# dphoyes/OpenCL-Structure-from-Motion

Hardware: AMD Instinct MI355X
Metric: stereo frame-pairs/sec (1242x375) through pushBack+matchFeatures(2), p_matched bit-exact (higher is better)
Workload: dtype u8

## Files before the change

### include/visomatch.h

```cpp
#ifndef VISOMATCH_H
#define VISOMATCH_H

#include <stdint.h>

#ifdef __cplusplus
extern "C" {
#endif

#define VSM_OK 0
#define VSM_EDIMS (-1)
#define VSM_ENOTREADY (-2)
#define VSM_EHIP (-3)
#define VSM_EARG (-4)

typedef struct vsm_handle vsm_handle;

typedef struct vsm_params {
  int32_t nms_n;
  int32_t nms_tau;
  int32_t match_binsize;
  int32_t match_radius;
  int32_t match_disp_tolerance;
  int32_t outlier_disp_tolerance;
  int32_t outlier_flow_tolerance;
// ... 155 lines not shown
int32_t vsm_host_ties(const int32_t *x, const int32_t *y, int32_t n, int32_t *pairs, int32_t cap);
int32_t vsm_debug_ties_gpu(const int32_t *x, const int32_t *y, int32_t n, int32_t *pairs, int32_t cap, double *kernel_us);

int32_t vsm_host_outliers_and_prior(const vsm_params *p, const vsm_p_match *list, int32_t n, int32_t method, vsm_p_match *out,
                                    int32_t cap, float *ranges, int32_t w, int32_t h);
int32_t vsm_host_outliers_and_prior_threads(const vsm_params *p, const vsm_p_match *list, int32_t n, int32_t method, vsm_p_match *out,
                                            int32_t cap, float *ranges, int32_t w, int32_t h, int32_t threads);
int32_t vsm_debug_dc2(const vsm_params *p, const vsm_p_match *list, int32_t n, int32_t method, int32_t gpu_ties, int32_t copies,
                      vsm_p_match *out, int32_t cap, float *ranges, int32_t w, int32_t h, double *kernel_us);
void vsm_debug_dc2_band_factor(int32_t f);
int32_t vsm_debug_predicates(const uint32_t *quads, int32_t n, int32_t *out);
int32_t vsm_debug_seq_plan(int32_t n_frames, int32_t pool_threads, int32_t host_in, int32_t seq_chunk, int32_t seq_first_chunk,
                           const char *plan, int32_t *chunk, int32_t *starts, int32_t cap);
int32_t vsm_debug_chunk_jobs(int32_t method, int32_t multi_stage, int32_t sides, int32_t banks, int32_t chunk, const int32_t *starts,
                             int32_t n_chunks, const int32_t *counts, const uint8_t *tr_valid, int32_t *frames_out, int32_t *max_nq_out);
int32_t vsm_debug_pair_jobs(int32_t method, int32_t multi_stage, int32_t sides, int32_t n_frames, const int32_t *counts, const int32_t *pairs,
                            int32_t n_pairs, int32_t chunk, const uint8_t *tr_valid, int32_t *pairs_out, int32_t *max_nq_out);
int32_t vsm_debug_refine(vsm_handle *h, int32_t method, const vsm_p_match *const *lists, const int32_t *counts, int32_t P,
                         vsm_p_match *const *out, int32_t *out_counts);
int32_t vsm_debug_refine_check(int32_t w, int32_t h, const vsm_p_match *const *lists, const int32_t *counts, int32_t P);
int32_t vsm_debug_parabolic_apply(const vsm_p_match *const *lists, const int32_t *const *records, const int32_t *counts, int32_t P,
                                  vsm_p_match *const *out, int32_t *out_counts);
int32_t vsm_host_parabolic_fits(const int32_t *records, int32_t n, float *uv, int32_t *ok);
int32_t vsm_debug_compact_keys(int32_t method, int32_t pass, int32_t P, const int32_t *n_query, const int32_t *const *flag,
                               const vsm_p_match *const *raw, const int32_t *key_cap, int32_t old_keys, vsm_p_match *const *list_out,
                               int32_t *count_out, uint64_t *const *keys_out);

typedef struct {
  vsm_params match;
  int32_t bucket_max_features;
  double bucket_width, bucket_height;
  double f, cu, cv;
  double base;
  int32_t ransac_iters;
  double inlier_threshold;
  int32_t reweighting;
} vsm_vo_stereo_params;
typedef struct vsm_vo_stereo vsm_vo_stereo;

void vsm_vo_stereo_default_params(vsm_vo_stereo_params *p);
vsm_vo_stereo *vsm_vo_stereo_create(const vsm_vo_stereo_params *p);
void vsm_vo_stereo_destroy(vsm_vo_stereo *v);
int vsm_vo_stereo_process(vsm_vo_stereo *v, const uint8_t *I1, const uint8_t *I2, int32_t width, int32_t height,
                          int32_t bpl, int replace);
int vsm_vo_stereo_process_device(vsm_vo_stereo *v, const uint8_t *dI1, const uint8_t *dI2, int32_t width,
                                 int32_t height, int32_t bpl, int replace);
// ... 88 lines not shown
```

### opencl-structure-from-motion_amd/csrc/vsm_api.cpp

```cpp
#include <math.h>
#include <stdio.h>
#include <stdlib.h>
#include <string.h>

#include <algorithm>
#include <chrono>
#include <memory>
#include <thread>
#include <unordered_map>
#include <vector>

#include "vsm_host.h"
#include "vsm_dc_gpu.h"
#include "vsm_internal.h"
#include "vsm_jobs.h"
#include "vsm_stage.h"
#include "vsm_tracks.h"
#include "vsm_points.h"
#include "vsm_resect.h"
#include "vsm_motions.h"

#define HIPCHK(expr)                                                                              \
  do {                                                                                            \
    hipError_t e_ = (expr);                                                                       \
    if (e_ != hipSuccess) {                                                                       \
      fprintf(stderr, "visomatch: HIP error %s at %s:%d (%s)\n", hipGetErrorString(e_), __FILE__, \
              __LINE__, #expr);                                                                   \
      return VSM_EHIP;                                                                            \
    }                                                                                             \
  } while (0)

static inline int32_t bpl16(int32_t w) { return w + 15 - (w - 1) % 16; }
static int cpu_budget() {
  unsigned hc = std::thread::hardware_concurrency();
  int budget = hc ? (int)hc : 8;
  if (FILE *f = fopen("/sys/fs/cgroup/cpu.max", "r")) {
    char q[64];
    long period = 0;
    if (fscanf(f, "%63s %ld", q, &period) == 2 && strcmp(q, "max") != 0 && period > 0) {
      long quota = atol(q);
      if (quota > 0) budget = std::min(budget, (int)std::max(1L, quota / period));
    }
    fclose(f);
// ... 1282 lines not shown
```

### opencl-structure-from-motion_amd/csrc/vsm_debug.inc

```

template <typename T>
struct DebugDev {
  T *p = nullptr;
  DebugDev() = default;
  DebugDev(const DebugDev &) = delete;
  DebugDev &operator=(const DebugDev &) = delete;
  ~DebugDev() {
    if (p) (void)hipFree(p);
  }
  bool alloc(size_t n) { return hipMalloc((void **)&p, std::max<size_t>(n, 1) * sizeof(T)) == hipSuccess; }
  operator T *() const { return p; }
};

struct DebugPairs {
  struct Pair {
    size_t raw = 0, flag = 0, blockcnt = 0, list1 = 0, list2 = 0, pf = 0;
    bool one_list = false;
    size_t keys = 0;
    int32_t key_cap = 0;
    int32_t count[2] = {0, 0};
    size_t n_in = 0;
    const vsm_p_match *raw_in = nullptr, *list2_in = nullptr;
    const int32_t *flag_in = nullptr, *pf_in = nullptr;
  };
// ... 623 lines not shown
int32_t vsm_debug_parabolic_apply(const vsm_p_match *const *lists, const int32_t *const *records, const int32_t *counts, int32_t P,
                                  vsm_p_match *const *out, int32_t *out_counts) {
  if (P < 1 || P > VSM_DEBUG_REFINE_MAX_PAIRS || !lists || !records || !counts || !out || !out_counts) return VSM_EARG;
  for (int32_t k = 0; k < P; k++)
    if (counts[k] < 0 || counts[k] > VSM_PARA_MAX_LIST || (counts[k] > 0 && (!lists[k] || !records[k]))) return VSM_EARG;
  DebugPairs D;
  HIPCHK(debug_lists_create(D, nullptr, lists, records, counts, P, true, VsmJob()));
  vsm_launch_parabolic_apply(nullptr, g_no_prof, D.d_pairs, P);
  HIPCHK(hipGetLastError());
  HIPCHK(hipDeviceSynchronize());
  HIPCHK(debug_lists_fetch(D, counts, P, true, out, out_counts));
  return VSM_OK;
}

int32_t vsm_host_parabolic_fits(const int32_t *records, int32_t n, float *uv, int32_t *ok) {
  if (n < 0 || (n > 0 && (!records || !uv || !ok))) return VSM_EARG;
  for (int32_t i = 0; i < n; i++) {
    const int32_t *r = records + (size_t)i * 12;
    ok[i] = vsm_host_parabolic_update(r + 3, r[1], r[2], uv[2 * i], uv[2 * i + 1]) ? 1 : 0;
  }
  return n;
}

}
```

### opencl-structure-from-motion_amd/csrc/vsm_dev.h

```cpp
#pragma once

#include "vsm_internal.h"

#define WAVE 64

#define VSM_AS1 __attribute__((address_space(1)))
typedef uint32_t vsm_u4 __attribute__((ext_vector_type(4)));
typedef int32_t vsm_i4 __attribute__((ext_vector_type(4)));
__device__ __forceinline__ uint4 ldg_u4(const void *p) {
  const vsm_u4 v = *(const VSM_AS1 vsm_u4 *)p;
  return make_uint4(v.x, v.y, v.z, v.w);
}
__device__ __forceinline__ int4 ldg_i4(const void *p) {
  const vsm_i4 v = *(const VSM_AS1 vsm_i4 *)p;
  return make_int4(v.x, v.y, v.z, v.w);
}
__device__ __forceinline__ uint4 ldg_u4_at(const void *base, uint32_t byte_off) {
  const vsm_u4 v = *(const VSM_AS1 vsm_u4 *)((const VSM_AS1 char *)base + byte_off);
  return make_uint4(v.x, v.y, v.z, v.w);
}
typedef uint32_t vsm_u4_a4 __attribute__((ext_vector_type(4), aligned(4)));
__device__ __forceinline__ uint4 ldg_u4_at_dw(const void *base, uint32_t byte_off) {
  const vsm_u4_a4 v = *(const VSM_AS1 vsm_u4_a4 *)((const VSM_AS1 char *)base + byte_off);
  return make_uint4(v.x, v.y, v.z, v.w);
}
__device__ __forceinline__ uint32_t ldg_u32_at(const void *base, uint32_t byte_off) {
  return *(const VSM_AS1 uint32_t *)((const VSM_AS1 char *)base + byte_off);
}
__device__ __forceinline__ int32_t ldg_i32(const void *p) { return *(const VSM_AS1 int32_t *)p; }
__device__ __forceinline__ uint32_t ldg_u32(const void *p) { return *(const VSM_AS1 uint32_t *)p; }

__device__ __forceinline__ int xcd_remap(int b, int nblocks) {
  const int per = (nblocks + 7) >> 3;
  return (b & 7) * per + (b >> 3);
// ... 53 lines not shown
```

### opencl-structure-from-motion_amd/csrc/vsm_match.hip

```cpp

#include <stdlib.h>

#include <algorithm>

#include "vsm_internal.h"
#include "vsm_dev.h"

#define VSM_MATCH_BLOCK 256
#define VSM_MATCH_WAVES 5
#define VSM_MATCH_GBIG 2
#define VSM_STEREO_BY_BIN 1

#ifdef VSM_MATCH_TIMING
#if VSM_MATCH_TIMING != 1 && VSM_MATCH_TIMING != 3
#error "VSM_MATCH_TIMING: 1 (cycles per stage and phase) or 3 (wave life on the device-wide clock)"
#endif
__device__ unsigned int vsm_mt_n;
__device__ unsigned int vsm_mt[1 << 18][8];
extern "C" int vsm_debug_match_timing(unsigned int *out, unsigned int cap, int reset) {
  unsigned int n = 0;
  if (hipMemcpyFromSymbol(&n, HIP_SYMBOL(vsm_mt_n), 4) != hipSuccess) return -1;
  if (n > (1u << 18)) n = 1u << 18;
  if (n > cap) n = cap;
  if (n && hipMemcpyFromSymbol(out, HIP_SYMBOL(vsm_mt), (size_t)n * 32) != hipSuccess) return -1;
  if (reset) {
    const unsigned int z = 0;
    if (hipMemcpyToSymbol(HIP_SYMBOL(vsm_mt_n), &z, 4) != hipSuccess) return -1;
  }
  return (int)n;
}
#if VSM_MATCH_TIMING == 1
#define MT_PHASE(k) const long long mt_ph##k = clock64()
#define MT_PHASE_ADD(ph)           \
// ... 587 lines not shown
}

__device__ __forceinline__ uint4 small_desc_tiled(const uint8_t *__restrict__ t, int bpl, int u, int v) {
#define TDU(x, y) ((uint32_t)t[vsm_tiled_at(bpl, (x), (y))])
#define TDV(x, y) ((uint32_t)t[vsm_tiled_at(bpl, (x), (y)) + VSM_TILED_DV])
  uint4 r;
  r.x = TDU(u, v - 2) | (TDU(u - 2, v - 1) << 8) | (TDU(u, v - 1) << 16) | (TDU(u + 2, v - 1) << 24);
  r.y = TDU(u - 1, v) | (TDU(u, v) << 8) | (TDU(u, v) << 16) | (TDU(u + 1, v) << 24);
  r.z = TDU(u - 2, v + 1) | (TDU(u, v + 1) << 8) | (TDU(u + 2, v + 1) << 16) | (TDU(u, v + 2) << 24);
  r.w = TDV(u, v - 1) | (TDV(u - 1, v) << 8) | (TDV(u + 1, v) << 16) | (TDV(u, v + 1) << 24);
#undef TDU
#undef TDV
  return r;
}

__device__ __forceinline__ uint32_t sad16(const uint4 &a, const uint4 &b) {
  uint32_t s = __builtin_amdgcn_sad_u8(a.x, b.x, 0u);
  s = __builtin_amdgcn_sad_u8(a.y, b.y, s);
  s = __builtin_amdgcn_sad_u8(a.z, b.z, s);
  return __builtin_amdgcn_sad_u8(a.w, b.w, s);
}

template <bool TILED>
__device__ __forceinline__ uint4 refine_ref_desc(const VsmImage &ref, const VsmDims &dc, int ru, int rv) {
  uint4 rd;
  const int b0 = (ru - 2) & ~3, rsh = 8 * ((ru - 2) - b0);
  uint64_t wu[5], wv[3];
  if (TILED) {
    const int j0 = b0 >> 2;
#pragma unroll
    for (int r = 0; r < 5; r++) {
      const uint8_t *row = ref.duv_tiled;
      const uint32_t lo = ldg_u32(row + vsm_tiled_at(dc.bpl, 4 * j0, rv - 2 + r)), hi = ldg_u32(row + vsm_tiled_at(dc.bpl, 4 * j0 + 4, rv - 2 + r));
      wu[r] = ((((uint64_t)hi) << 32) | lo) >> rsh;
      if (r >= 1 && r <= 3) {
        const uint32_t lv = ldg_u32(row + vsm_tiled_at(dc.bpl, 4 * j0, rv - 2 + r) + VSM_TILED_DV), hv = ldg_u32(row + vsm_tiled_at(dc.bpl, 4 * j0 + 4, rv - 2 + r) + VSM_TILED_DV);
        wv[r - 1] = ((((uint64_t)hv) << 32) | lv) >> rsh;
      }
    }
  } else {
#pragma unroll
    for (int r = 0; r < 5; r++) {
      const uint32_t *pr = (const uint32_t *)(ref.du_full + (size_t)(rv - 2 + r) * dc.bpl + b0);
      wu[r] = ((((uint64_t)pr[1]) << 32) | pr[0]) >> rsh;
    }
#pragma unroll
    for (int r = 0; r < 3; r++) {
      const uint32_t *pr = (const uint32_t *)(ref.dv_full + (size_t)(rv - 1 + r) * dc.bpl + b0);
      wv[r] = ((((uint64_t)pr[1]) << 32) | pr[0]) >> rsh;
    }
  }
#define WB(w, c) ((uint32_t)((w) >> (8 * (c))) & 0xffu)
  rd.x = WB(wu[0], 2) | (WB(wu[1], 0) << 8) | (WB(wu[1], 2) << 16) | (WB(wu[1], 4) << 24);
  rd.y = WB(wu[2], 1) | (WB(wu[2], 2) << 8) | (WB(wu[2], 2) << 16) | (WB(wu[2], 3) << 24);
  rd.z = WB(wu[3], 0) | (WB(wu[3], 2) << 8) | (WB(wu[3], 4) << 16) | (WB(wu[4], 2) << 24);
  rd.w = WB(wv[0], 2) | (WB(wv[1], 1) << 8) | (WB(wv[1], 3) << 16) | (WB(wv[2], 2) << 24);
#undef WB
  return rd;
}

template <bool TILED>
__global__ void __launch_bounds__(256)
    k_refine(const VsmImage *__restrict__ imgs, const VsmPair *__restrict__ pairs, const VsmJob *__restrict__ jobs,
             VsmJob job0, VsmDims dp, VsmDims dc, int method, int nbx, int npairs) {
  const int lb = xcd_remap(blockIdx.x, gridDim.x);
  const int pj = lb / nbx, bx = lb - pj * nbx;
  if (pj >= npairs) return;
  const VsmJob &jb = jobs ? jobs[pj] : job0;
  const VsmPair &pair = pairs[pj];
  const int g = bx * blockDim.x + threadIdx.x;
  const int mi = g / 3, step = g - mi * 3;
  const VsmImage &ref = imgs[jb.img_curr];
  uint4 rd;
  {
    const int lane = threadIdx.x & 63;
    const int first_mi = (g - lane) / 3, rmi = first_mi + lane;
    uint4 mine = make_uint4(0, 0, 0, 0);
    if (lane < 22 && rmi < pair.count[1]) {
      const vsm_p_match *rm = pair.list2 + rmi;
      mine = refine_ref_desc<TILED>(ref, dc, (int)rm->u1c, (int)rm->v1c);
    }
    const int src = mi - first_mi;
    rd.x = (uint32_t)__shfl((int)mine.x, src, 64);
    rd.y = (uint32_t)__shfl((int)mine.y, src, 64);
    rd.z = (uint32_t)__shfl((int)mine.z, src, 64);
    rd.w = (uint32_t)__shfl((int)mine.w, src, 64);
  }
  if (mi >= pair.count[1]) return;
  if (step == 0 && !(method == 0 || method == 2)) return;
  if (step == 1 && !(method == 1 || method == 2)) return;
  if (step == 2 && method != 2) return;
  vsm_p_match *m = pair.list2 + mi;
  const VsmImage &tgt = step == 0 ? imgs[jb.img_prev] : (step == 1 ? imgs[jb.img_curr + 1] : imgs[jb.img_prev + 1]);
  const VsmDims &dt = step == 1 ? dc : dp;
  float *pu = step == 0 ? &m->u1p : (step == 1 ? &m->u2c : &m->u2p);
  float *pv = pu + 1;
  const float u2 = *pu, v2 = *pv;
  if (u2 - 2 < VSM_MARGIN || u2 + 2 > dt.w - 1 - VSM_MARGIN || v2 - 2 < VSM_MARGIN || v2 + 2 > dt.h - 1 - VSM_MARGIN)
    return;
  const int iu = (int)u2, iv = (int)v2;
  uint32_t U[9][3], V[9][3];
  if (TILED) {
    const int o = (iu - 4) & 7, b = o >> 2;
    const uint32_t sb = (uint32_t)(o & 3);
#pragma unroll
    for (int r = 0; r < 9; r++) {
      const uint8_t *pr = tgt.duv_tiled + vsm_tiled_at(dt.bpl, (iu - 4) & ~7, iv - 4 + r);
      const uint4 t0 = ldg_u4(pr), t1 = ldg_u4(pr + 128);
      const uint32_t d0 = b ? t0.z : t0.x, d1 = b ? t1.x : t0.z, d2 = b ? t1.z : t1.x;
      U[r][0] = __builtin_amdgcn_alignbyte(d1, d0, sb);
      U[r][1] = __builtin_amdgcn_alignbyte(d2, d1, sb);
      U[r][2] = d2 >> (8 * sb);
      const uint32_t e0 = b ? t0.w : t0.y, e1 = b ? t1.y : t0.w, e2 = b ? t1.w : t1.y;
      V[r][0] = __builtin_amdgcn_alignbyte(e1, e0, sb);
      V[r][1] = __builtin_amdgcn_alignbyte(e2, e1, sb);
      V[r][2] = e2 >> (8 * sb);
    }
  } else {
    const int a0 = (iu - 4) & ~3, sh = 8 * ((iu - 4) - a0);
#pragma unroll
    for (int r = 0; r < 9; r++) {
      const uint32_t *pr = (const uint32_t *)(tgt.du_full + (size_t)(iv - 4 + r) * dt.bpl + a0);
      const uint32_t d0 = pr[0], d1 = pr[1], d2 = pr[2];
      U[r][0] = (uint32_t)((((uint64_t)d1 << 32) | d0) >> sh);
      U[r][1] = (uint32_t)((((uint64_t)d2 << 32) | d1) >> sh);
      U[r][2] = d2 >> sh;
      if (r >= 1 && r <= 7) {
        const uint32_t *qr = (const uint32_t *)(tgt.dv_full + (size_t)(iv - 4 + r) * dt.bpl + a0);
        const uint32_t e0 = qr[0], e1 = qr[1], e2 = qr[2];
        V[r][0] = (uint32_t)((((uint64_t)e1 << 32) | e0) >> sh);
        V[r][1] = (uint32_t)((((uint64_t)e2 << 32) | e1) >> sh);
        V[r][2] = e2 >> sh;
      } else {
        V[r][0] = V[r][1] = V[r][2] = 0;
      }
    }
  }
#define UB(r, c) ((U[(r)][(c) >> 2] >> (8 * ((c)&3))) & 0xffu)
#define VB(r, c) ((V[(r)][(c) >> 2] >> (8 * ((c)&3))) & 0xffu)
  uint32_t best = 0xffffffffu;
  int ind = 0;
#pragma unroll
  for (int ddv = 0; ddv < 5; ddv++) {
#pragma unroll
    for (int ddu = 0; ddu < 5; ddu++) {
      const int r = ddv + 2, c = ddu + 2;
      uint4 t;
      t.x = UB(r - 2, c) | (UB(r - 1, c - 2) << 8) | (UB(r - 1, c) << 16) | (UB(r - 1, c + 2) << 24);
      t.y = UB(r, c - 1) | (UB(r, c) << 8) | (UB(r, c) << 16) | (UB(r, c + 1) << 24);
      t.z = UB(r + 1, c - 2) | (UB(r + 1, c) << 8) | (UB(r + 1, c + 2) << 16) | (UB(r + 2, c) << 24);
      t.w = VB(r - 1, c) | (VB(r, c - 1) << 8) | (VB(r, c + 1) << 16) | (VB(r + 1, c) << 24);
      const uint32_t cost = sad16(rd, t);
      if (cost < best) {
        best = cost;
        ind = ddv * 5 + ddu;
      }
    }
  }
#undef UB
#undef VB
  *pu = (float)((double)u2 + ((double)(float)(ind % 5) - 2.0));
  *pv = (float)((double)v2 + ((double)(float)(ind / 5) - 2.0));
}

__global__ void __launch_bounds__(256)
    k_parabolic_costs(const VsmImage *__restrict__ imgs, const VsmPair *__restrict__ pairs,
                      const VsmJob *__restrict__ jobs, VsmJob job0, VsmDims dp, VsmDims dc, int method) {
  const VsmJob &jb = jobs ? jobs[blockIdx.y] : job0;
  const VsmPair &pair = pairs[blockIdx.y];
  const int img_prev = jb.img_prev, img_curr = jb.img_curr;
  const int lane = threadIdx.x & 63;
  const int g = (blockIdx.x * blockDim.x + threadIdx.x) >> 6;
  const int mi = g / 3, step = g - mi * 3;
  if (mi >= pair.count[1]) return;
  int32_t *out = pair.pf + ((size_t)mi * 3 + step) * 12;
  bool active = !((step == 0 && !(method == 0 || method == 2)) || (step == 1 && !(method == 1 || method == 2)) ||
                  (step == 2 && method != 2));
  if (!active) {
    if (lane == 0) out[0] = 2;
    return;
  }
  const vsm_p_match *m = pair.list2 + mi;
  const VsmImage &ref = imgs[img_curr];
  const VsmImage &tgt = step == 0 ? imgs[img_prev] : (step == 1 ? imgs[img_curr + 1] : imgs[img_prev + 1]);
  const VsmDims &dt = step == 1 ? dc : dp;
// ... 259 lines not shown

void vsm_launch_export_xy(hipStream_t s, const VsmPair *d_pairs, uint32_t *dst_host_mapped, int n_upper) {
  hipLaunchKernelGGL(k_export_xy, dim3(max(min(cdiv(n_upper, 256), 64), 1)), dim3(256), 0, s, d_pairs, dst_host_mapped);
}

void vsm_launch_parabolic_apply(hipStream_t s, VsmProf &pf, const VsmPair *d_pairs, int npairs) {
  if (npairs <= 0) return;
  static const VsmParaPlan plan = make_para_plan();
  pf.begin(VSM_K_PARA_APPLY, s);
  hipLaunchKernelGGL(k_parabolic_apply, dim3(npairs), dim3(1024), 0, s, d_pairs, plan);
  pf.end(s);
}

void vsm_launch_refine(hipStream_t s, VsmProf &pf, const VsmImage *d_imgs, const VsmPair *d_pairs, const VsmJob *d_jobs,
                       const VsmJob &job0, int npairs, const VsmDims &dp, const VsmDims &dc, int method, int refinement,
                       int n_upper) {
  if (n_upper <= 0) return;
  pf.begin(VSM_K_REFINE, s);
  if (refinement == 2)
    hipLaunchKernelGGL(k_parabolic_costs, dim3(cdiv(n_upper * 3 * 64, 256), npairs), dim3(256), 0, s, d_imgs, d_pairs,
                       d_jobs, job0, dp, dc, method);
  else
  {
    const int nbx = cdiv(n_upper * 3, 256), tot = ((nbx * npairs + 7) / 8) * 8;
    if (dc.scale == 2)
      hipLaunchKernelGGL(k_refine<true>, dim3(tot), dim3(256), 0, s, d_imgs, d_pairs, d_jobs, job0, dp, dc, method, nbx, npairs);
    else
      hipLaunchKernelGGL(k_refine<false>, dim3(tot), dim3(256), 0, s, d_imgs, d_pairs, d_jobs, job0, dp, dc, method, nbx, npairs);
  }
  pf.end(s);
}
```

### opencl-structure-from-motion_amd/visomatch.py

```python
import ctypes as C
import os

import numpy as np

HERE = os.path.dirname(os.path.abspath(__file__))
os.environ.setdefault("GPU_MAX_HW_QUEUES", "5")
LIB_PATH = os.environ.get("VSM_LIB_PATH") or os.path.join(HERE, "libvisomatch.so")

P_MATCH = np.dtype(
    [("u1p", "<f4"), ("v1p", "<f4"), ("i1p", "<i4"), ("u2p", "<f4"), ("v2p", "<f4"), ("i2p", "<i4"),
     ("u1c", "<f4"), ("v1c", "<f4"), ("i1c", "<i4"), ("u2c", "<f4"), ("v2c", "<f4"), ("i2c", "<i4")])
assert P_MATCH.itemsize == 48

INT_PARAMS = ["nms_n", "nms_tau", "match_binsize", "match_radius", "match_disp_tolerance",
              "outlier_disp_tolerance", "outlier_flow_tolerance", "multi_stage", "half_resolution", "refinement"]
TRACKS_WAVE_MAX = 64
TRACKS_BLOCK_MAX = 2048
FEATURE_SETS = {"1p1": 0, "2p1": 1, "1c1": 2, "2c1": 3, "1p2": 4, "2p2": 5, "1c2": 6, "2c2": 7}

EXPORTS = ["vsm_default_params", "vsm_create", "vsm_destroy", "vsm_set_intrinsics", "vsm_push_back",
           "vsm_push_back_device", "vsm_wait_for_stream", "vsm_match", "vsm_num_matches", "vsm_get_matches", "vsm_bucket", "vsm_gain",
           "vsm_num_features", "vsm_get_features", "vsm_set_stage_capture", "vsm_stage_size", "vsm_stage_get",
           "vsm_num_ranges", "vsm_get_ranges", "vsm_get_gradients", "vsm_get_filter_responses", "vsm_get_counters",
           "vsm_get_timings", "vsm_set_profiling", "vsm_num_kernels", "vsm_kernel_name", "vsm_get_kernel_stats",
           "vsm_host_delaunay", "vsm_host_delaunay_split", "vsm_debug_delaunay_gpu", "vsm_debug_dc_bench", "vsm_host_ties", "vsm_debug_ties_gpu", "vsm_host_outliers_and_prior", "vsm_host_outliers_and_prior_threads", "vsm_debug_dc2", "vsm_debug_dc2_band_factor", "vsm_debug_predicates", "vsm_debug_seq_plan", "vsm_debug_chunk_jobs", "vsm_debug_pair_jobs", "vsm_debug_refine", "vsm_debug_refine_check", "vsm_debug_parabolic_apply", "vsm_host_parabolic_fits", "vsm_debug_compact_keys", "vsm_local_cpus", "vsm_forkjoin_cpus", "vsm_device_pool_stats", "vsm_device_pool_trim", "vsm_sequence_run", "vsm_sequence_num_matches", "vsm_sequence_get_matches",
           "vsm_sequence_get_timings", "vsm_sequence_path", "vsm_pairs_run", "vsm_pairs_num_matches", "vsm_pairs_get_matches", "vsm_pairs_get_timings",
           "vsm_tracks_run", "vsm_pairs_tracks", "vsm_tracks_count", "vsm_tracks_num_obs", "vsm_tracks_get", "vsm_tracks_of_matches",
           "vsm_tracks_get_stats", "vsm_tracks_get_timings", "vsm_host_tracks",
           "vsm_triangulate_default_params", "vsm_triangulate_run", "vsm_tracks_triangulate", "vsm_points_count", "vsm_points_get",
           "vsm_points_get_stats", "vsm_points_get_timings", "vsm_host_triangulate",
           "vsm_resect_default_params", "vsm_resect_run", "vsm_points_resect", "vsm_resect_count", "vsm_resect_get", "vsm_resect_get_stats",
           "vsm_resect_get_timings", "vsm_host_resect", "vsm_set_option", "vsm_version", "vsm_host_register", "vsm_host_unregister",
           "vsm_multi_create", "vsm_multi_destroy", "vsm_multi_process", "vsm_multi_num_sequences", "vsm_multi_get_motion",
           "vsm_multi_motion_valid", "vsm_multi_num_matches", "vsm_multi_get_matches", "vsm_multi_num_inliers", "vsm_multi_get_inliers",
           "vsm_multi_get_timings",
           "vsm_vo_stereo_default_params", "vsm_vo_stereo_create", "vsm_vo_stereo_destroy", "vsm_vo_stereo_process",
           "vsm_vo_stereo_process_device", "vsm_vo_stereo_process_matches", "vsm_vo_stereo_get_motion",
           "vsm_vo_stereo_motion_valid", "vsm_vo_stereo_num_matches", "vsm_vo_stereo_get_matches",
           "vsm_vo_stereo_num_inliers", "vsm_vo_stereo_get_inliers", "vsm_vo_stereo_gain", "vsm_vo_stereo_matcher",
           "vsm_vo_stereo_get_timings", "vsm_vo_sampler_seed", "vsm_host_estimate_motion_stereo",
           "vsm_vo_mono_default_params", "vsm_vo_mono_create", "vsm_vo_mono_destroy", "vsm_vo_mono_process",
           "vsm_vo_mono_process_device", "vsm_vo_mono_process_matches", "vsm_vo_mono_get_motion",
           "vsm_vo_mono_motion_valid", "vsm_vo_mono_num_matches", "vsm_vo_mono_get_matches", "vsm_vo_mono_num_inliers",
           "vsm_vo_mono_get_inliers", "vsm_vo_mono_gain", "vsm_vo_mono_matcher", "vsm_vo_mono_get_timings",
           "vsm_vo_mono_device_svd", "vsm_vo_mono_device_stages",
           "vsm_debug_mono_fit", "vsm_debug_mono_count", "vsm_debug_mono_triangulate", "vsm_debug_mono_vote",
           "vsm_host_estimate_motion_mono",
           "vsm_motions_run", "vsm_pairs_motions", "vsm_motions_count", "vsm_motions_get", "vsm_motions_inliers", "vsm_motions_matches",
# ... 106 lines not shown
        L.vsm_kernel_name.argtypes = [i32]
        L.vsm_get_kernel_stats.argtypes = [vp, vp, vp]
        L.vsm_host_delaunay.argtypes = [vp, vp, i32, vp, i32, i32]
        L.vsm_host_delaunay_split.argtypes = [vp, vp, i32, vp, i32, i32, i32]
        L.vsm_debug_delaunay_gpu.argtypes = [vp, vp, i32, vp, i32, i32, i32, i32]
        L.vsm_debug_dc_bench.argtypes = [vp, vp, i32, i32, i32, i32, i32, i32]
        L.vsm_debug_dc_bench.restype = C.c_double
        L.vsm_host_ties.argtypes = [vp, vp, i32, vp, i32]
        L.vsm_debug_ties_gpu.argtypes = [vp, vp, i32, vp, i32, vp]
        L.vsm_host_outliers_and_prior.argtypes = [C.POINTER(VsmParams), vp, i32, i32, vp, i32, vp, i32, i32]
        L.vsm_host_outliers_and_prior_threads.argtypes = [C.POINTER(VsmParams), vp, i32, i32, vp, i32, vp, i32, i32, i32]
        L.vsm_debug_dc2.argtypes = [C.POINTER(VsmParams), vp, i32, i32, i32, i32, vp, i32, vp, i32, i32, vp]
        L.vsm_debug_dc2_band_factor.argtypes = [i32]
        L.vsm_debug_predicates.argtypes = [vp, i32, vp]
        L.vsm_debug_seq_plan.argtypes = [i32, i32, i32, i32, i32, C.c_char_p, vp, vp, i32]
        L.vsm_debug_chunk_jobs.restype = i32
        L.vsm_debug_chunk_jobs.argtypes = [i32, i32, i32, i32, i32, vp, i32, vp, vp, vp, vp]
        L.vsm_debug_pair_jobs.restype = i32
        L.vsm_debug_pair_jobs.argtypes = [i32, i32, i32, i32, vp, vp, i32, i32, vp, vp, vp]
        L.vsm_debug_refine.argtypes = [vp, i32, vp, vp, i32, vp, vp]
        L.vsm_debug_refine_check.argtypes = [i32, i32, vp, vp, i32]
        L.vsm_debug_parabolic_apply.argtypes = [vp, vp, vp, i32, vp, vp]
        L.vsm_host_parabolic_fits.argtypes = [vp, i32, vp, vp]
        L.vsm_debug_compact_keys.argtypes = [i32, i32, i32, vp, vp, vp, vp, i32, vp, vp, vp]
        L.vsm_pairs_run.argtypes = [vp, vp, vp, C.c_int64, C.c_int, i32, i32, i32, i32, i32, vp, i32, vp, vp]
        L.vsm_pairs_num_matches.argtypes = [vp, i32]
        L.vsm_pairs_get_matches.argtypes = [vp, i32, vp, i32]
        L.vsm_pairs_get_timings.argtypes = [vp, vp]
        L.vsm_pairs_get_timings.restype = None
        L.vsm_tracks_run.argtypes = [vp, i32, vp, i32, vp, vp, i32, i32]
        L.vsm_pairs_tracks.argtypes = [vp, i32, i32]
        L.vsm_tracks_count.argtypes = [vp]
        L.vsm_tracks_num_obs.argtypes = [vp]
        L.vsm_tracks_get.argtypes = [vp, vp, vp, vp]
        L.vsm_tracks_of_matches.argtypes = [vp, i32, vp, i32]
        L.vsm_tracks_get_stats.argtypes = [vp, vp]
        L.vsm_tracks_get_stats.restype = None
        L.vsm_tracks_get_timings.argtypes = [vp, vp]
        L.vsm_tracks_get_timings.restype = None
        L.vsm_host_tracks.restype = i32
        L.vsm_host_tracks.argtypes = [i32, vp, i32, vp, vp, i32, i32, vp, vp, vp, vp, vp]
        f64 = C.c_double
        L.vsm_triangulate_default_params.argtypes = [C.POINTER(VsmTriangulateParams)]
        L.vsm_triangulate_default_params.restype = None
        L.vsm_triangulate_run.argtypes = [vp, i32, vp, vp, f64, f64, f64, i32, vp, vp, vp, vp, C.POINTER(VsmTriangulateParams)]
        L.vsm_tracks_triangulate.argtypes = [vp, vp, vp, vp, vp, f64, f64, f64, C.POINTER(VsmTriangulateParams)]
# ... 611 lines not shown


def device_parabolic_apply(lists, records, counts=None):
    ms, cnt, ptrs = _refine_inputs(lists)
    rs = [np.ascontiguousarray(r, dtype=np.int32).reshape(-1, 3, 12) for r in records]
    assert len(rs) == len(ms) and all(len(r) == len(m) for r, m in zip(rs, ms))
    rptrs = (C.c_void_p * max(len(rs), 1))(*[r.ctypes.data if len(r) else None for r in rs])
    if counts is not None:
        cnt = np.ascontiguousarray(counts, dtype=np.int32)
    outs, oc, optrs = _refine_outputs([len(m) for m in ms])
    _check(lib().vsm_debug_parabolic_apply(ptrs, rptrs, _ptr(cnt), len(ms), optrs, _ptr(oc)), "vsm_debug_parabolic_apply")
    return [o[:n].copy() for o, n in zip(outs, oc)]


def host_parabolic_fits(records, uv):
    r = np.ascontiguousarray(records, dtype=np.int32).reshape(-1, 12)
    out = np.array(uv, dtype=np.float32).reshape(-1, 2).copy()
    assert len(out) == len(r)
    ok = np.zeros(len(r), dtype=np.int32)
    _check(lib().vsm_host_parabolic_fits(_ptr(r), len(r), _ptr(out), _ptr(ok)), "vsm_host_parabolic_fits")
    return out, ok


COMPACT_KEY_GUARD = 8


def device_compact_keys(flags, raws, key_caps, method=2, pass_=1, old_keys=False):
    fs = [np.ascontiguousarray(f, dtype=np.int32) for f in flags]
    rs = [np.ascontiguousarray(r, dtype=P_MATCH) for r in raws]
    assert len(fs) == len(rs) == len(key_caps) and all(len(f) == len(r) for f, r in zip(fs, rs))
    nq = np.array([len(f) for f in fs], dtype=np.int32)
    caps = np.ascontiguousarray(key_caps, dtype=np.int32)
    lists = [np.zeros(len(f) + 1, dtype=P_MATCH) for f in fs]
    keys = [np.zeros(int(c) + COMPACT_KEY_GUARD, dtype=np.uint64) for c in caps]
    counts = np.full(len(fs), -1, dtype=np.int32)
    tab = lambda arrs: (C.c_void_p * len(arrs))(*[a.ctypes.data for a in arrs])
    _check(lib().vsm_debug_compact_keys(int(method), int(pass_), len(fs), _ptr(nq), tab(fs), tab(rs), _ptr(caps), int(old_keys), tab(lists),
                                        _ptr(counts), tab(keys)), "vsm_debug_compact_keys")
    return [(l, int(n), k) for l, n, k in zip(lists, counts, keys)]


def local_cpus():
    buf = (C.c_int32 * 1024)()
    n = lib().vsm_local_cpus(C.cast(buf, C.c_void_p), 1024)
    return [int(buf[i]) for i in range(min(n, 1024))]

# ... 640 lines not shown
```

Measured before the change: 55750.

## Restructure refine kernel into per-wave steps with shared reference descriptors

Rewrites k_refine so that each block handles 64 matches, with one wave per refinement step and an extra wave that builds the reference descriptor into shared memory. The old scheme used a thread per (match, step) and shuffled the reference descriptors across lanes. Descriptor assembly now uses byte-permute helpers in a shared header, and the costs are computed first with a packed key min-reduction. It also adds a host reference path for testing. The intent is to cut per-thread index math and divergence and to use fewer instructions for packing. The trade-offs are a __syncthreads, one whole wave per block spent only on the reference, and a waves_per_eu constraint.

```diff
diff --git a/include/visomatch.h b/include/visomatch.h
--- a/include/visomatch.h
+++ b/include/visomatch.h
@@ -201,6 +201,9 @@
 int32_t vsm_debug_parabolic_apply(const vsm_p_match *const *lists, const int32_t *const *records, const int32_t *counts, int32_t P,
                                   vsm_p_match *const *out, int32_t *out_counts);
 int32_t vsm_host_parabolic_fits(const int32_t *records, int32_t n, float *uv, int32_t *ok);
+int32_t vsm_host_refine_forms(const uint8_t *du, const uint8_t *dv, const uint8_t *ref_du, const uint8_t *ref_dv, const int32_t *phase,
+                              const int32_t *ref_phase, int32_t n, int32_t *costs, int32_t *index);
+int32_t vsm_debug_refine_group(void);
 int32_t vsm_debug_compact_keys(int32_t method, int32_t pass, int32_t P, const int32_t *n_query, const int32_t *const *flag,
                                const vsm_p_match *const *raw, const int32_t *key_cap, int32_t old_keys, vsm_p_match *const *list_out,
                                int32_t *count_out, uint64_t *const *keys_out);
diff --git a/opencl-structure-from-motion_amd/csrc/vsm_api.cpp b/opencl-structure-from-motion_amd/csrc/vsm_api.cpp
--- a/opencl-structure-from-motion_amd/csrc/vsm_api.cpp
+++ b/opencl-structure-from-motion_amd/csrc/vsm_api.cpp
@@ -19,6 +19,7 @@
 #include "vsm_points.h"
 #include "vsm_resect.h"
 #include "vsm_motions.h"
+#include "vsm_refine.h"
 
 #define HIPCHK(expr)                                                                              \
   do {                                                                                            \
diff --git a/opencl-structure-from-motion_amd/csrc/vsm_debug.inc b/opencl-structure-from-motion_amd/csrc/vsm_debug.inc
--- a/opencl-structure-from-motion_amd/csrc/vsm_debug.inc
+++ b/opencl-structure-from-motion_amd/csrc/vsm_debug.inc
@@ -669,4 +669,32 @@
   return n;
 }
 
-}
+int32_t vsm_debug_refine_group(void) { return VR_GROUP; }
+
+int32_t vsm_host_refine_forms(const uint8_t *du, const uint8_t *dv, const uint8_t *ref_du, const uint8_t *ref_dv, const int32_t *phase,
+                              const int32_t *ref_phase, int32_t n, int32_t *costs, int32_t *index) {
+  if (n < 0 || (n > 0 && (!du || !dv || !ref_du || !ref_dv || !phase || !ref_phase || !costs || !index))) return VSM_EARG;
+  for (int32_t i = 0; i < n; i++)
+    if (phase[i] < 0 || phase[i] > 7 || ref_phase[i] < 0 || ref_phase[i] > 3) return VSM_EARG;
+  auto dword = [](const uint8_t *p) { return (uint32_t)p[0] | ((uint32_t)p[1] << 8) | ((uint32_t)p[2] << 16) | ((uint32_t)p[3] << 24); };
+  for (int32_t i = 0; i < n; i++) {
+    uint32_t U[9][3], V[9][3], RU[5][3], RV[5][3];
+    for (int r = 0; r < 9; r++) {
+      const uint8_t *pu = du + ((size_t)i * 9 + r) * 16, *pv = dv + ((size_t)i * 9 + r) * 16;
+      const uint32_t t0[4] = {dword(pu), dword(pv), dword(pu + 4), dword(pv + 4)}, t1[4] = {dword(pu + 8), dword(pv + 8), dword(pu + 12), dword(pv + 12)};
+      vr_tile_row(t0, t1, phase[i], U[r], V[r]);
+    }
+    for (int r = 0; r < 5; r++) {
+      const uint8_t *pu = ref_du + ((size_t)i * 5 + r) * 8, *pv = ref_dv + ((size_t)i * 5 + r) * 8;
+      vr_ref_row(dword(pu), dword(pu + 4), (uint32_t)ref_phase[i], RU[r]);
+      vr_ref_row(dword(pv), dword(pv + 4), (uint32_t)ref_phase[i], RV[r]);
+    }
+    uint32_t cost[25];
+    vr_costs(U, V, vr_ref_desc(RU, RV), cost);
+    for (int k = 0; k < 25; k++) costs[(size_t)i * 25 + k] = (int32_t)cost[k];
+    index[i] = vr_first_min(cost);
+  }
+  return n;
+}
+
+}
diff --git a/opencl-structure-from-motion_amd/csrc/vsm_dev.h b/opencl-structure-from-motion_amd/csrc/vsm_dev.h
--- a/opencl-structure-from-motion_amd/csrc/vsm_dev.h
+++ b/opencl-structure-from-motion_amd/csrc/vsm_dev.h
@@ -10,6 +10,11 @@
 __device__ __forceinline__ uint4 ldg_u4(const void *p) {
   const vsm_u4 v = *(const VSM_AS1 vsm_u4 *)p;
   return make_uint4(v.x, v.y, v.z, v.w);
+}
+typedef uint32_t vsm_u2 __attribute__((ext_vector_type(2)));
+__device__ __forceinline__ uint2 ldg_u2_at(const void *base, uint32_t byte_off) {
+  const vsm_u2 v = *(const VSM_AS1 vsm_u2 *)((const VSM_AS1 char *)base + byte_off);
+  return make_uint2(v.x, v.y);
 }
 __device__ __forceinline__ int4 ldg_i4(const void *p) {
   const vsm_i4 v = *(const VSM_AS1 vsm_i4 *)p;
diff --git a/opencl-structure-from-motion_amd/csrc/vsm_match.hip b/opencl-structure-from-motion_amd/csrc/vsm_match.hip
--- a/opencl-structure-from-motion_amd/csrc/vsm_match.hip
+++ b/opencl-structure-from-motion_amd/csrc/vsm_match.hip
@@ -5,10 +5,12 @@
 
 #include "vsm_internal.h"
 #include "vsm_dev.h"
+#include "vsm_refine.h"
 
 #define VSM_MATCH_BLOCK 256
 #define VSM_MATCH_WAVES 5
 #define VSM_MATCH_GBIG 2
+#define VSM_REFINE_WAVES 5
 #define VSM_STEREO_BY_BIN 1
 
 #ifdef VSM_MATCH_TIMING
@@ -642,145 +644,112 @@
 }
 
 template <bool TILED>
-__device__ __forceinline__ uint4 refine_ref_desc(const VsmImage &ref, const VsmDims &dc, int ru, int rv) {
-  uint4 rd;
-  const int b0 = (ru - 2) & ~3, rsh = 8 * ((ru - 2) - b0);
-  uint64_t wu[5], wv[3];
+__device__ __forceinline__ VrDesc refine_reference(const VsmImage &ref, const VsmDims &dc, int ru, int rv) {
+  const int b0 = (ru - 2) & ~3;
+  const uint32_t sb = (uint32_t)((ru - 2) - b0);
+  uint32_t U[5][3], V[5][3];
   if (TILED) {
-    const int j0 = b0 >> 2;
 #pragma unroll
     for (int r = 0; r < 5; r++) {
-      const uint8_t *row = ref.duv_tiled;
-      const uint32_t lo = ldg_u32(row + vsm_tiled_at(dc.bpl, 4 * j0, rv - 2 + r)), hi = ldg_u32(row + vsm_tiled_at(dc.bpl, 4 * j0 + 4, rv - 2 + r));
-      wu[r] = ((((uint64_t)hi) << 32) | lo) >> rsh;
-      if (r >= 1 && r <= 3) {
-        const uint32_t lv = ldg_u32(row + vsm_tiled_at(dc.bpl, 4 * j0, rv - 2 + r) + VSM_TILED_DV), hv = ldg_u32(row + vsm_tiled_at(dc.bpl, 4 * j0 + 4, rv - 2 + r) + VSM_TILED_DV);
-        wv[r - 1] = ((((uint64_t)hv) << 32) | lv) >> rsh;
-      }
+      const uint2 lo = ldg_u2_at(ref.duv_tiled, (uint32_t)vsm_tiled_at(dc.bpl, b0, rv - 2 + r)),
+                  hi = ldg_u2_at(ref.duv_tiled, (uint32_t)vsm_tiled_at(dc.bpl, b0 + 4, rv - 2 + r));
+      vr_ref_row(lo.x, hi.x, sb, U[r]);
+      vr_ref_row(lo.y, hi.y, sb, V[r]);
     }
   } else {
 #pragma unroll
     for (int r = 0; r < 5; r++) {
-      const uint32_t *pr = (const uint32_t *)(ref.du_full + (size_t)(rv - 2 + r) * dc.bpl + b0);
-      wu[r] = ((((uint64_t)pr[1]) << 32) | pr[0]) >> rsh;
-    }
-#pragma unroll
-    for (int r = 0; r < 3; r++) {
-      const uint32_t *pr = (const uint32_t *)(ref.dv_full + (size_t)(rv - 1 + r) * dc.bpl + b0);
-      wv[r] = ((((uint64_t)pr[1]) << 32) | pr[0]) >> rsh;
-    }
-  }
-#define WB(w, c) ((uint32_t)((w) >> (8 * (c))) & 0xffu)
-  rd.x = WB(wu[0], 2) | (WB(wu[1], 0) << 8) | (WB(wu[1], 2) << 16) | (WB(wu[1], 4) << 24);
-  rd.y = WB(wu[2], 1) | (WB(wu[2], 2) << 8) | (WB(wu[2], 2) << 16) | (WB(wu[2], 3) << 24);
-  rd.z = WB(wu[3], 0) | (WB(wu[3], 2) << 8) | (WB(wu[3], 4) << 16) | (WB(wu[4], 2) << 24);
-  rd.w = WB(wv[0], 2) | (WB(wv[1], 1) << 8) | (WB(wv[1], 3) << 16) | (WB(wv[2], 2) << 24);
-#undef WB
-  return rd;
+      const uint32_t at = (uint32_t)((rv - 2 + r) * dc.bpl + b0);
+      vr_ref_row(ldg_u32_at(ref.du_full, at), ldg_u32_at(ref.du_full, at + 4), sb, U[r]);
+      if (r >= 1 && r <= 3)
+        vr_ref_row(ldg_u32_at(ref.dv_full, at), ldg_u32_at(ref.dv_full, at + 4), sb, V[r]);
+      else
+        V[r][0] = V[r][1] = V[r][2] = 0;
+    }
+  }
+  return vr_ref_desc(U, V);
 }
 
 template <bool TILED>
-__global__ void __launch_bounds__(256)
+__device__ __forceinline__ void refine_window(const VsmImage &tgt, int bpl, int iu, int iv, uint32_t (&U)[9][3], uint32_t (&V)[9][3]) {
+  if (TILED) {
+    const int o = (iu - 4) & 7;
+    uint4 t0[9], t1[9];
+#pragma unroll
+    for (int r = 0; r < 9; r++) {
+      const uint32_t at = (uint32_t)vsm_tiled_at(bpl, (iu - 4) & ~7, iv - 4 + r);
+      t0[r] = ldg_u4_at(tgt.duv_tiled, at), t1[r] = ldg_u4_at(tgt.duv_tiled, at + 128);
+    }
+    __builtin_amdgcn_sched_barrier(0);
+#pragma unroll
+    for (int r = 0; r < 9; r++) {
+      const uint32_t a[4] = {t0[r].x, t0[r].y, t0[r].z, t0[r].w}, b[4] = {t1[r].x, t1[r].y, t1[r].z, t1[r].w};
+      vr_tile_row(a, b, o, U[r], V[r]);
+    }
+  } else {
+    const int a0 = (iu - 4) & ~3;
+    const uint32_t sb = (uint32_t)((iu - 4) - a0);
+#pragma unroll
+    for (int r = 0; r < 9; r++) {
+      const uint32_t at = (uint32_t)((iv - 4 + r) * bpl + a0);
+      vr_window_row(ldg_u32_at(tgt.du_full, at), ldg_u32_at(tgt.du_full, at + 4), ldg_u32_at(tgt.du_full, at + 8), sb, U[r]);
+      if (r >= 1 && r <= 7)
+        vr_window_row(ldg_u32_at(tgt.dv_full, at), ldg_u32_at(tgt.dv_full, at + 4), ldg_u32_at(tgt.dv_full, at + 8), sb, V[r]);
+      else
+        V[r][0] = V[r][1] = V[r][2] = 0;
+    }
+  }
+}
+
+template <bool TILED>
+__global__ void __launch_bounds__(256) __attribute__((amdgpu_waves_per_eu(VSM_REFINE_WAVES, VSM_REFINE_WAVES)))
     k_refine(const VsmImage *__restrict__ imgs, const VsmPair *__restrict__ pairs, const VsmJob *__restrict__ jobs,
              VsmJob job0, VsmDims dp, VsmDims dc, int method, int nbx, int npairs) {
+  __shared__ uint4 s_rd[VR_GROUP];
   const int lb = xcd_remap(blockIdx.x, gridDim.x);
   const int pj = lb / nbx, bx = lb - pj * nbx;
   if (pj >= npairs) return;
-  const VsmJob &jb = jobs ? jobs[pj] : job0;
+  const int img_prev = jobs ? jobs[pj].img_prev : job0.img_prev, img_curr = jobs ? jobs[pj].img_curr : job0.img_curr;
   const VsmPair &pair = pairs[pj];
-  const int g = bx * blockDim.x + threadIdx.x;
-  const int mi = g / 3, step = g - mi * 3;
-  const VsmImage &ref = imgs[jb.img_curr];
-  uint4 rd;
-  {
-    const int lane = threadIdx.x & 63;
-    const int first_mi = (g - lane) / 3, rmi = first_mi + lane;
-    uint4 mine = make_uint4(0, 0, 0, 0);
-    if (lane < 22 && rmi < pair.count[1]) {
-      const vsm_p_match *rm = pair.list2 + rmi;
-      mine = refine_ref_desc<TILED>(ref, dc, (int)rm->u1c, (int)rm->v1c);
-    }
-    const int src = mi - first_mi;
-    rd.x = (uint32_t)__shfl((int)mine.x, src, 64);
-    rd.y = (uint32_t)__shfl((int)mine.y, src, 64);
-    rd.z = (uint32_t)__shfl((int)mine.z, src, 64);
-    rd.w = (uint32_t)__shfl((int)mine.w, src, 64);
-  }
-  if (mi >= pair.count[1]) return;
-  if (step == 0 && !(method == 0 || method == 2)) return;
-  if (step == 1 && !(method == 1 || method == 2)) return;
-  if (step == 2 && method != 2) return;
-  vsm_p_match *m = pair.list2 + mi;
-  const VsmImage &tgt = step == 0 ? imgs[jb.img_prev] : (step == 1 ? imgs[jb.img_curr + 1] : imgs[jb.img_prev + 1]);
-  const VsmDims &dt = step == 1 ? dc : dp;
-  float *pu = step == 0 ? &m->u1p : (step == 1 ? &m->u2c : &m->u2p);
-  float *pv = pu + 1;
-  const float u2 = *pu, v2 = *pv;
-  if (u2 - 2 < VSM_MARGIN || u2 + 2 > dt.w - 1 - VSM_MARGIN || v2 - 2 < VSM_MARGIN || v2 + 2 > dt.h - 1 - VSM_MARGIN)
-    return;
-  const int iu = (int)u2, iv = (int)v2;
+  const int count = pair.count[1];
+  if (bx * VR_GROUP >= count) return;
+  const int lane = threadIdx.x & 63, wv = __builtin_amdgcn_readfirstlane(threadIdx.x >> 6);
+  const int nsteps = method == 2 ? 3 : 1;
+  const int step = method == 2 ? wv : method;
+  const int mi = bx * VR_GROUP + lane;
+  const bool live = mi < count;
+  vsm_p_match *m = pair.list2 + (live ? mi : count - 1);
+  float u2 = 0.f, v2 = 0.f;
+  bool ok = false;
   uint32_t U[9][3], V[9][3];
-  if (TILED) {
-    const int o = (iu - 4) & 7, b = o >> 2;
-    const uint32_t sb = (uint32_t)(o & 3);
-#pragma unroll
-    for (int r = 0; r < 9; r++) {
-      const uint8_t *pr = tgt.duv_tiled + vsm_tiled_at(dt.bpl, (iu - 4) & ~7, iv - 4 + r);
-      const uint4 t0 = ldg_u4(pr), t1 = ldg_u4(pr + 128);
-      const uint32_t d0 = b ? t0.z : t0.x, d1 = b ? t1.x : t0.z, d2 = b ? t1.z : t1.x;
-      U[r][0] = __builtin_amdgcn_alignbyte(d1, d0, sb);
-      U[r][1] = __builtin_amdgcn_alignbyte(d2, d1, sb);
-      U[r][2] = d2 >> (8 * sb);
-      const uint32_t e0 = b ? t0.w : t0.y, e1 = b ? t1.y : t0.w, e2 = b ? t1.w : t1.y;
-      V[r][0] = __builtin_amdgcn_alignbyte(e1, e0, sb);
-      V[r][1] = __builtin_amdgcn_alignbyte(e2, e1, sb);
-      V[r][2] = e2 >> (8 * sb);
-    }
+  if (wv == nsteps) {
+    const uint4 p1 = ldg_u4((const uint8_t *)m + 16);
+    const VrDesc d = refine_reference<TILED>(imgs[img_curr], dc, (int)__uint_as_float(p1.z), (int)__uint_as_float(p1.w));
+    s_rd[lane] = make_uint4(d.a0, d.b, d.a1, d.x);
   } else {
-    const int a0 = (iu - 4) & ~3, sh = 8 * ((iu - 4) - a0);
-#pragma unroll
-    for (int r = 0; r < 9; r++) {
-      const uint32_t *pr = (const uint32_t *)(tgt.du_full + (size_t)(iv - 4 + r) * dt.bpl + a0);
-      const uint32_t d0 = pr[0], d1 = pr[1], d2 = pr[2];
-      U[r][0] = (uint32_t)((((uint64_t)d1 << 32) | d0) >> sh);
-      U[r][1] = (uint32_t)((((uint64_t)d2 << 32) | d1) >> sh);
-      U[r][2] = d2 >> sh;
-      if (r >= 1 && r <= 7) {
-        const uint32_t *qr = (const uint32_t *)(tgt.dv_full + (size_t)(iv - 4 + r) * dt.bpl + a0);
-        const uint32_t e0 = qr[0], e1 = qr[1], e2 = qr[2];
-        V[r][0] = (uint32_t)((((uint64_t)e1 << 32) | e0) >> sh);
-        V[r][1] = (uint32_t)((((uint64_t)e2 << 32) | e1) >> sh);
-        V[r][2] = e2 >> sh;
-      } else {
-        V[r][0] = V[r][1] = V[r][2] = 0;
-      }
-    }
-  }
-#define UB(r, c) ((U[(r)][(c) >> 2] >> (8 * ((c)&3))) & 0xffu)
-#define VB(r, c) ((V[(r)][(c) >> 2] >> (8 * ((c)&3))) & 0xffu)
-  uint32_t best = 0xffffffffu;
-  int ind = 0;
-#pragma unroll
-  for (int ddv = 0; ddv < 5; ddv++) {
-#pragma unroll
-    for (int ddu = 0; ddu < 5; ddu++) {
-      const int r = ddv + 2, c = ddu + 2;
-      uint4 t;
-      t.x = UB(r - 2, c) | (UB(r - 1, c - 2) << 8) | (UB(r - 1, c) << 16) | (UB(r - 1, c + 2) << 24);
-      t.y = UB(r, c - 1) | (UB(r, c) << 8) | (UB(r, c) << 16) | (UB(r, c + 1) << 24);
-      t.z = UB(r + 1, c - 2) | (UB(r + 1, c) << 8) | (UB(r + 1, c + 2) << 16) | (UB(r + 2, c) << 24);
-      t.w = VB(r - 1, c) | (VB(r, c - 1) << 8) | (VB(r, c + 1) << 16) | (VB(r + 1, c) << 24);
-      const uint32_t cost = sad16(rd, t);
-      if (cost < best) {
-        best = cost;
-        ind = ddv * 5 + ddu;
-      }
-    }
-  }
-#undef UB
-#undef VB
-  *pu = (float)((double)u2 + ((double)(float)(ind % 5) - 2.0));
-  *pv = (float)((double)v2 + ((double)(float)(ind / 5) - 2.0));
+    if (step == 1) {
+      const uint4 p2 = ldg_u4((const uint8_t *)m + 32);
+      u2 = __uint_as_float(p2.y), v2 = __uint_as_float(p2.z);
+    } else {
+      const uint4 p0 = ldg_u4((const uint8_t *)m), p1 = ldg_u4((const uint8_t *)m + 16);
+      u2 = __uint_as_float(step == 0 ? p0.x : p0.w), v2 = __uint_as_float(step == 0 ? p0.y : p1.x);
+    }
+    const int tw = step == 1 ? dc.w : dp.w, th = step == 1 ? dc.h : dp.h, tbpl = step == 1 ? dc.bpl : dp.bpl;
+    ok = !(u2 - 2 < VSM_MARGIN || u2 + 2 > tw - 1 - VSM_MARGIN || v2 - 2 < VSM_MARGIN || v2 + 2 > th - 1 - VSM_MARGIN);
+    if (ok) refine_window<TILED>(imgs[step == 0 ? img_prev : (step == 1 ? img_curr + 1 : img_prev + 1)], tbpl, (int)u2, (int)v2, U, V);
+  }
+  __syncthreads();
+  if (wv == nsteps) return;
+  const uint4 q = s_rd[lane];
+  const VrDesc rd = {q.x, q.y, q.z, q.w};
+  uint32_t cost[25];
+  vr_costs(U, V, rd, cost);
+  const int ind = vr_first_min(cost);
+  if (live && ok) {
+    float *pu = step == 0 ? &m->u1p : (step == 1 ? &m->u2c : &m->u2p);
+    pu[0] = (float)((double)u2 + ((double)(float)(ind % 5) - 2.0));
+    pu[1] = (float)((double)v2 + ((double)(float)(ind / 5) - 2.0));
+  }
 }
 
 __global__ void __launch_bounds__(256)
@@ -1086,11 +1055,11 @@
                        d_jobs, job0, dp, dc, method);
   else
   {
-    const int nbx = cdiv(n_upper * 3, 256), tot = ((nbx * npairs + 7) / 8) * 8;
+    const int nbx = cdiv(n_upper, VR_GROUP), tot = ((nbx * npairs + 7) / 8) * 8, threads = 64 * ((method == 2 ? 3 : 1) + 1);
     if (dc.scale == 2)
-      hipLaunchKernelGGL(k_refine<true>, dim3(tot), dim3(256), 0, s, d_imgs, d_pairs, d_jobs, job0, dp, dc, method, nbx, npairs);
+      hipLaunchKernelGGL(k_refine<true>, dim3(tot), dim3(threads), 0, s, d_imgs, d_pairs, d_jobs, job0, dp, dc, method, nbx, npairs);
     else
-      hipLaunchKernelGGL(k_refine<false>, dim3(tot), dim3(256), 0, s, d_imgs, d_pairs, d_jobs, job0, dp, dc, method, nbx, npairs);
+      hipLaunchKernelGGL(k_refine<false>, dim3(tot), dim3(threads), 0, s, d_imgs, d_pairs, d_jobs, job0, dp, dc, method, nbx, npairs);
   }
   pf.end(s);
 }
diff --git a/opencl-structure-from-motion_amd/csrc/vsm_refine.h b/opencl-structure-from-motion_amd/csrc/vsm_refine.h
--- /dev/null
+++ b/opencl-structure-from-motion_amd/csrc/vsm_refine.h
@@ -0,0 +1,104 @@
+#pragma once
+
+#include "vsm_feat.h"
+
+#define VR_GROUP 64
+
+VF_HD uint32_t vr_sad(uint32_t a, uint32_t b, uint32_t acc) {
+#if defined(__HIP_DEVICE_COMPILE__)
+  return __builtin_amdgcn_sad_u8(a, b, acc);
+#else
+  for (int k = 0; k < 4; k++) {
+    const int x = (int)((a >> (8 * k)) & 0xffu), y = (int)((b >> (8 * k)) & 0xffu);
+    acc += (uint32_t)(x > y ? x - y : y - x);
+  }
+  return acc;
+#endif
+}
+
+struct VrDesc {
+  uint32_t a0, b, a1, x;
+};
+
+VF_HD void vr_window_row(uint32_t d0, uint32_t d1, uint32_t d2, uint32_t sb, uint32_t (&W)[3]) {
+  W[0] = vf_alignbyte(d1, d0, sb);
+  W[1] = vf_alignbyte(d2, d1, sb);
+  W[2] = d2 >> (8 * sb);
+}
+
+VF_HD void vr_tile_row(const uint32_t (&t0)[4], const uint32_t (&t1)[4], int o, uint32_t (&U)[3], uint32_t (&V)[3]) {
+  const bool b = (o >> 2) != 0;
+  const uint32_t sb = (uint32_t)(o & 3);
+  vr_window_row(b ? t0[2] : t0[0], b ? t1[0] : t0[2], b ? t1[2] : t1[0], sb, U);
+  vr_window_row(b ? t0[3] : t0[1], b ? t1[1] : t0[3], b ? t1[3] : t1[1], sb, V);
+}
+
+VF_HD void vr_ref_row(uint32_t lo, uint32_t hi, uint32_t sb, uint32_t (&W)[3]) {
+  W[0] = vf_alignbyte(hi, lo, sb);
+  W[1] = hi >> (8 * sb);
+  W[2] = 0;
+}
+
+VF_HD uint32_t vr_pick(const uint32_t (&W)[3], int c0, int c1, int c2, int c3) {
+#define VR_DW(c) ((c) < 0 ? 2 : (c) >> 2)
+#define VR_SEL(c, k) (((c) < 0 ? 0x0cu : (uint32_t)((c)-4 * lo)) << (8 * (k)))
+  const int l01 = VR_DW(c0) < VR_DW(c1) ? VR_DW(c0) : VR_DW(c1), l23 = VR_DW(c2) < VR_DW(c3) ? VR_DW(c2) : VR_DW(c3);
+  const int lo = l01 < l23 ? l01 : l23;
+  const uint32_t sel = VR_SEL(c0, 0) | VR_SEL(c1, 1) | VR_SEL(c2, 2) | VR_SEL(c3, 3);
+#undef VR_DW
+#undef VR_SEL
+  return lo == 0 ? vf_perm(W[1], W[0], sel) : (lo == 1 ? vf_perm(W[2], W[1], sel) : vf_perm(W[2], W[2], sel));
+}
+
+template <int ROWS>
+VF_HD uint32_t vr_form_a(const uint32_t (&U)[ROWS][3], const uint32_t (&V)[ROWS][3], int R, int c) {
+  return vf_perm(V[R][c >> 2], vr_pick(U[R], c - 2, c, c + 2, -1), 0x00020100u | ((uint32_t)(4 + (c & 3)) << 24));
+}
+template <int ROWS>
+VF_HD uint32_t vr_form_b(const uint32_t (&U)[ROWS][3], int R, int c) {
+  return vr_pick(U[R], c - 1, c, c, c + 1);
+}
+template <int ROWS>
+VF_HD uint32_t vr_form_x(const uint32_t (&U)[ROWS][3], const uint32_t (&V)[ROWS][3], int r, int c) {
+  const uint32_t col = (uint32_t)(c & 3);
+  return vf_perm(U[r + 2][c >> 2], U[r - 2][c >> 2], 0x0c0c0000u | ((4 + col) << 8) | col) | vr_pick(V[r], -1, -1, c - 1, c + 1);
+}
+
+template <int ROWS>
+VF_HD VrDesc vr_desc(const uint32_t (&U)[ROWS][3], const uint32_t (&V)[ROWS][3], int r, int c) {
+  VrDesc d;
+  d.a0 = vr_form_a<ROWS>(U, V, r - 1, c);
+  d.b = vr_form_b<ROWS>(U, r, c);
+  d.a1 = vr_form_a<ROWS>(U, V, r + 1, c);
+  d.x = vr_form_x<ROWS>(U, V, r, c);
+  return d;
+}
+
+VF_HD VrDesc vr_ref_desc(const uint32_t (&U)[5][3], const uint32_t (&V)[5][3]) { return vr_desc<5>(U, V, 2, 2); }
+
+VF_HD void vr_costs(const uint32_t (&U)[9][3], const uint32_t (&V)[9][3], const VrDesc &rd, uint32_t (&cost)[25]) {
+#if defined(__HIP_DEVICE_COMPILE__)
+#pragma unroll
+#endif
+  for (int ddv = 0; ddv < 5; ddv++) {
+#if defined(__HIP_DEVICE_COMPILE__)
+#pragma unroll
+#endif
+    for (int ddu = 0; ddu < 5; ddu++) {
+      const VrDesc t = vr_desc<9>(U, V, ddv + 2, ddu + 2);
+      cost[ddv * 5 + ddu] = vr_sad(rd.x, t.x, vr_sad(rd.a1, t.a1, vr_sad(rd.b, t.b, vr_sad(rd.a0, t.a0, 0u))));
+    }
+  }
+}
+
+VF_HD int vr_first_min(const uint32_t (&cost)[25]) {
+  uint32_t best = 0xffffffffu;
+#if defined(__HIP_DEVICE_COMPILE__)
+#pragma unroll
+#endif
+  for (int k = 0; k < 25; k++) {
+    const uint32_t key = (cost[k] << 5) | (uint32_t)k;
+    best = key < best ? key : best;
+  }
+  return (int)(best & 31u);
+}
diff --git a/opencl-structure-from-motion_amd/visomatch.py b/opencl-structure-from-motion_amd/visomatch.py
--- a/opencl-structure-from-motion_amd/visomatch.py
+++ b/opencl-structure-from-motion_amd/visomatch.py
@@ -23,7 +23,7 @@
            "vsm_num_features", "vsm_get_features", "vsm_set_stage_capture", "vsm_stage_size", "vsm_stage_get",
            "vsm_num_ranges", "vsm_get_ranges", "vsm_get_gradients", "vsm_get_filter_responses", "vsm_get_counters",
            "vsm_get_timings", "vsm_set_profiling", "vsm_num_kernels", "vsm_kernel_name", "vsm_get_kernel_stats",
-           "vsm_host_delaunay", "vsm_host_delaunay_split", "vsm_debug_delaunay_gpu", "vsm_debug_dc_bench", "vsm_host_ties", "vsm_debug_ties_gpu", "vsm_host_outliers_and_prior", "vsm_host_outliers_and_prior_threads", "vsm_debug_dc2", "vsm_debug_dc2_band_factor", "vsm_debug_predicates", "vsm_debug_seq_plan", "vsm_debug_chunk_jobs", "vsm_debug_pair_jobs", "vsm_debug_refine", "vsm_debug_refine_check", "vsm_debug_parabolic_apply", "vsm_host_parabolic_fits", "vsm_debug_compact_keys", "vsm_local_cpus", "vsm_forkjoin_cpus", "vsm_device_pool_stats", "vsm_device_pool_trim", "vsm_sequence_run", "vsm_sequence_num_matches", "vsm_sequence_get_matches",
+           "vsm_host_delaunay", "vsm_host_delaunay_split", "vsm_debug_delaunay_gpu", "vsm_debug_dc_bench", "vsm_host_ties", "vsm_debug_ties_gpu", "vsm_host_outliers_and_prior", "vsm_host_outliers_and_prior_threads", "vsm_debug_dc2", "vsm_debug_dc2_band_factor", "vsm_debug_predicates", "vsm_debug_seq_plan", "vsm_debug_chunk_jobs", "vsm_debug_pair_jobs", "vsm_debug_refine", "vsm_debug_refine_check", "vsm_debug_parabolic_apply", "vsm_host_parabolic_fits", "vsm_host_refine_forms", "vsm_debug_refine_group", "vsm_debug_compact_keys", "vsm_local_cpus", "vsm_forkjoin_cpus", "vsm_device_pool_stats", "vsm_device_pool_trim", "vsm_sequence_run", "vsm_sequence_num_matches", "vsm_sequence_get_matches",
            "vsm_sequence_get_timings", "vsm_sequence_path", "vsm_pairs_run", "vsm_pairs_num_matches", "vsm_pairs_get_matches", "vsm_pairs_get_timings",
            "vsm_tracks_run", "vsm_pairs_tracks", "vsm_tracks_count", "vsm_tracks_num_obs", "vsm_tracks_get", "vsm_tracks_of_matches",
            "vsm_tracks_get_stats", "vsm_tracks_get_timings", "vsm_host_tracks",
@@ -176,6 +176,8 @@
         L.vsm_debug_refine_check.argtypes = [i32, i32, vp, vp, i32]
         L.vsm_debug_parabolic_apply.argtypes = [vp, vp, vp, i32, vp, vp]
         L.vsm_host_parabolic_fits.argtypes = [vp, i32, vp, vp]
+        L.vsm_host_refine_forms.argtypes = [vp, vp, vp, vp, vp, vp, i32, vp, vp]
+        L.vsm_debug_refine_group.argtypes = []
         L.vsm_debug_compact_keys.argtypes = [i32, i32, i32, vp, vp, vp, vp, i32, vp, vp, vp]
         L.vsm_pairs_run.argtypes = [vp, vp, vp, C.c_int64, C.c_int, i32, i32, i32, i32, i32, vp, i32, vp, vp]
         L.vsm_pairs_num_matches.argtypes = [vp, i32]
@@ -833,6 +835,33 @@
     return out, ok
 
 
+def refine_group():
+    return int(lib().vsm_debug_refine_group())
+
+
+def host_refine_forms(du, dv, ref_du, ref_dv, phase, ref_phase):
+    du, dv, ref_du, ref_dv = (np.ascontiguousarray(a, dtype=np.uint8) for a in (du, dv, ref_du, ref_dv))
+    n = len(du)
+    phase = np.ascontiguousarray(phase, dtype=np.int32)
+    ref_phase = np.ascontiguousarray(ref_phase, dtype=np.int32)
+    assert du.shape == dv.shape == (n, 9, 9) and ref_du.shape == ref_dv.shape == (n, 5, 5) and phase.shape == ref_phase.shape == (n,)
+    i = np.arange(n)[:, None, None]
+    rows = []
+    for a, ph, width in ((du, phase, 16), (dv, phase, 16), (ref_du, ref_phase, 8), (ref_dv, ref_phase, 8)):
+        k = a.shape[1]
+        wide = ((np.arange(n * k * width).reshape(n, k, width) * 37 + 11) % 256).astype(np.uint8)
+        if n and (ph.min() < 0 or ph.max() + k > width):
+            wide = np.ascontiguousarray(wide)
+        else:
+            wide[i, np.arange(k)[None, :, None], ph[:, None, None] + np.arange(k)[None, None, :]] = a
+        rows.append(np.ascontiguousarray(wide))
+    costs = np.zeros((n, 25), dtype=np.int32)
+    index = np.zeros(n, dtype=np.int32)
+    _check(lib().vsm_host_refine_forms(_ptr(rows[0]), _ptr(rows[1]), _ptr(rows[2]), _ptr(rows[3]), _ptr(phase), _ptr(ref_phase), n, _ptr(costs), _ptr(index)),
+           "vsm_host_refine_forms")
+    return costs, index
+
+
 COMPACT_KEY_GUARD = 8
 
 
```

Measured after the change: 55500. About the same (-0.5%).
